# mirsadm/motioncam-decoder

Hardware: AMD Instinct MI355X
Metric: MPixels/s unpacked + achieved HBM GB/s %peak, 4K 12-bit, 1/2/4/8 GPUs (higher is better)
Workload: dtype u16; 1 GPU; 3840x2160 12-bit type-7 x 240 frames/GPU, Nat (smooth field + noise sigma 12); frames_per_gpu=240, width=3840, height=2160, bits=12, encoding=7, streams=1

## Files before the change

### motioncam_decoder_amd/csrc/mcraw_dev.h

```cpp
#pragma once
#include <hip/hip_runtime.h>
#include <stdint.h>

#include "mcraw_plan.h"

namespace mcraw {

typedef unsigned short u16x2 __attribute__((ext_vector_type(2)));

__device__ __forceinline__ uint32_t len7_of(uint32_t b)
{
    return b <= 6u ? 8u * b : (b <= 8u ? 64u : (b <= 10u ? 80u : 128u));
}

__device__ __forceinline__ uint32_t cls7_of(uint32_t b)
{
    return b <= 6u ? b : (b <= 8u ? 7u : (b <= 10u ? 8u : 9u));
}

__device__ __forceinline__ uint32_t byte_mask(uint32_t g)
{
    return __builtin_amdgcn_perm(0u, 0u, 0x0C0C0C0Cu + g);
}

// ... 110 lines not shown

__device__ __forceinline__ void post_pack12(const uint32_t p[4], uint32_t o[3])
{
    uint32_t t[4];
#pragma unroll
    for (int i = 0; i < 4; i++) {
        const uint32_t c = __builtin_bit_cast(uint32_t, __builtin_elementwise_min(__builtin_bit_cast(mcraw_u16x2, p[i]),
                                                                                  __builtin_bit_cast(mcraw_u16x2, 0x0FFF0FFFu)));
        t[i] = __builtin_amdgcn_udot2(__builtin_bit_cast(mcraw_u16x2, c), __builtin_bit_cast(mcraw_u16x2, 0x00011000u), 0u, false);
    }
    o[0] = __builtin_amdgcn_perm(t[1], t[0], 0x06000102u);
    o[1] = __builtin_amdgcn_perm(t[2], t[1], 0x05060001u);
    o[2] = __builtin_amdgcn_perm(t[3], t[2], 0x04050600u);
}

__device__ __forceinline__ void post_pack12_lean(const uint32_t p[4], uint32_t o[3])
{
    uint32_t t[4];
#pragma unroll
    for (int i = 0; i < 4; i++)
        t[i] = __builtin_amdgcn_udot2(__builtin_bit_cast(mcraw_u16x2, p[i]), __builtin_bit_cast(mcraw_u16x2, 0x00011000u), 0u, false);
    o[0] = __builtin_amdgcn_perm(t[1], t[0], 0x06000102u);
    o[1] = __builtin_amdgcn_perm(t[2], t[1], 0x05060001u);
    o[2] = __builtin_amdgcn_perm(t[3], t[2], 0x04050600u);
}

template <int B, bool CLAMP>
__device__ __forceinline__ void post_pack_be(const uint32_t p[4], uint32_t o[4])
{
    static_assert(B == 10 || B == 14, "strip rows of 10 or 14 bits per sample");
    constexpr uint32_t MAXV = (1u << B) - 1u;
    uint32_t g[4];
#pragma unroll
    for (int i = 0; i < 4; i++) {
        uint32_t c = p[i];
        if (CLAMP)
            c = __builtin_bit_cast(uint32_t, __builtin_elementwise_min(__builtin_bit_cast(mcraw_u16x2, c), __builtin_bit_cast(mcraw_u16x2, MAXV | (MAXV << 16))));
        g[i] = __builtin_amdgcn_udot2(__builtin_bit_cast(mcraw_u16x2, c), __builtin_bit_cast(mcraw_u16x2, 0x00010000u | (1u << B)), 0u, false);
    }
    uint32_t w[4];
    if (B == 10) {
        w[0] = (g[0] << 12) | (g[1] >> 8);
        w[1] = (g[1] << 24) | (g[2] << 4) | (g[3] >> 16);
        w[2] = g[3] << 16;
        w[3] = 0u;
    } else {
        w[0] = (g[0] << 4) | (g[1] >> 24);
        w[1] = (g[1] << 8) | (g[2] >> 20);
        w[2] = (g[2] << 12) | (g[3] >> 16);
        w[3] = g[3] << 16;
    }
#pragma unroll
    for (int i = 0; i < 4; i++)
        o[i] = __builtin_amdgcn_perm(w[i], w[i], 0x00010203u);
}

#define MCRAW_GLOBAL __attribute__((address_space(1)))
template <class V, class T>
__device__ __forceinline__ MCRAW_GLOBAL V *gptr(T *p)
{
    return (MCRAW_GLOBAL V *)p;
}

#ifndef MCRAW_STORE_POLICY
#define MCRAW_STORE_POLICY "sc1 nt"
#endif
typedef uint32_t mcraw_u32x4 __attribute__((ext_vector_type(4)));
typedef uint32_t mcraw_u32x3 __attribute__((ext_vector_type(3)));
#if defined(__HIP_DEVICE_COMPILE__) && !defined(__gfx950__) && !defined(__gfx942__)
#error "store_stream16/12: the `sc1 nt` mnemonics and the two wait states behind a store of more than 8 bytes are gfx940+ facts"
#endif
__device__ __forceinline__ void store_stream16(void *dst, mcraw_u32x4 v)
{
    asm volatile("global_store_dwordx4 %0, %1, off " MCRAW_STORE_POLICY "\n\ts_nop 1" ::"v"(dst), "v"(v) : "memory");
}
__device__ __forceinline__ void store_stream12(void *dst, mcraw_u32x3 v)
{
    asm volatile("global_store_dwordx3 %0, %1, off " MCRAW_STORE_POLICY "\n\ts_nop 1" ::"v"(dst), "v"(v) : "memory");
}
typedef uint32_t mcraw_u32x2 __attribute__((ext_vector_type(2)));
__device__ __forceinline__ void store_stream8(void *dst, mcraw_u32x2 v)
{
    asm volatile("global_store_dwordx2 %0, %1, off " MCRAW_STORE_POLICY ::"v"(dst), "v"(v) : "memory");
}

enum StorePath {
    SP_ALIGNED,
    SP_UNALIGNED,
    SP_CROPPED,
    SP_MERGED_FWD,
    SP_MERGED_BACK,
};
#ifndef MCRAW_STORE_PATH
#define MCRAW_STORE_PATH(form, cond)
#endif

__device__ __forceinline__ void post_store_bytes(uint8_t *dst, const uint32_t *o, uint32_t nb, uint32_t last, uint32_t maxb)
{
    for (uint32_t i = 0; i < maxb; i++)
        if (i < nb) {
            uint32_t b = (o[i >> 2] >> (8u * (i & 3u))) & 0xffu;
            if (i == nb - 1u)
                b &= last;
            gptr<uint8_t>(dst)[i] = static_cast<uint8_t>(b);
        }
}

template <bool NT, int PB>
__device__ __forceinline__ void post_store8(uint16_t *out, const Post &post, uint32_t width, uint32_t y, uint32_t x,
                                            uint32_t p[4], uint32_t n, bool quick, bool lean = false)
{
    if (!(PB != 16 && lean) && (post.mode & POST_BLACK))
        post_black(p, post, y);
    if (PB == 10 || PB == 14) {
        constexpr uint32_t B = PB == 10 ? 10u : 14u;
        uint32_t o[4];
        if (lean)
            post_pack_be<(PB == 10 ? 10 : 14), false>(p, o);
        else
            post_pack_be<(PB == 10 ? 10 : 14), true>(p, o);
        uint8_t *dst = reinterpret_cast<uint8_t *>(out) + static_cast<size_t>(y) * post_row_bytes(width, post.mode) + (x >> 3) * B;
        if (quick && n == 8u) {
            MCRAW_STORE_PATH(SP_ALIGNED, true);
            typedef uint32_t u32x2_u __attribute__((ext_vector_type(2), aligned(2)));
            typedef uint32_t u32x3_u __attribute__((ext_vector_type(3), aligned(2)));
            if (PB == 10) {
                const u32x2_u v = {o[0], o[1]};
                *gptr<u32x2_u>(dst) = v;
                *gptr<uint16_t>(dst + 8) = static_cast<uint16_t>(o[2]);
            } else {
                const u32x3_u v = {o[0], o[1], o[2]};
                *gptr<u32x3_u>(dst) = v;
                *gptr<uint16_t>(dst + 12) = static_cast<uint16_t>(o[3]);
            }
        } else {
            MCRAW_STORE_PATH(SP_UNALIGNED, n == 8u);
            MCRAW_STORE_PATH(SP_CROPPED, n != 8u);
            const uint32_t bitsn = n * B, nb = (bitsn + 7u) >> 3;
            post_store_bytes(dst, o, nb, (bitsn & 7u) ? (0xffu << (8u - (bitsn & 7u))) & 0xffu : 0xffu, 14u);
        }
        return;
    }
    if (PB == 12) {
        uint32_t o[3];
        if (lean)
            post_pack12_lean(p, o);
        else
            post_pack12(p, o);
        uint8_t *dst = reinterpret_cast<uint8_t *>(out) + static_cast<size_t>(y) * post_row_bytes(width, post.mode) + (x >> 3) * 12u;
        if (quick && n == 8u) {
            MCRAW_STORE_PATH(SP_ALIGNED, true);
            typedef uint32_t u32x3 __attribute__((ext_vector_type(3), aligned(4)));
            const u32x3 v = {o[0], o[1], o[2]};
            if (NT)
                store_stream12(dst, v);
            else
                *gptr<u32x3>(dst) = v;
        } else if (n == 8u) {
            MCRAW_STORE_PATH(SP_UNALIGNED, true);
            typedef uint32_t u32x3_u __attribute__((ext_vector_type(3), aligned(1)));
            const u32x3_u v = {o[0], o[1], o[2]};
            *gptr<u32x3_u>(dst) = v;
        } else {
            MCRAW_STORE_PATH(SP_CROPPED, true);
            const uint32_t nb = (n * 12u + 7u) >> 3;
#pragma unroll
// ... 190 lines not shown
```

### motioncam_decoder_amd/csrc/mcraw_type7.hip

```cpp
#include <algorithm>
#include <cstdlib>

#if defined(MCRAW_PATHST) || defined(MCRAW_PATHS7)
#include "mcraw_census.h"
#endif
#ifdef MCRAW_PATHST
namespace mcraw {
enum PathT {
    PT_WAVES,
    PT_INVALID,
    PT_SHORT,
    PT_TILES_SKIPPED,
    PT_SPAN_EMPTY, PT_SPAN_FULL, PT_HEAD,
    PT_WG_REMAP, PT_WG_CHUNKED,
    PT_CLS0, PT_CLS9 = PT_CLS0 + 9,
    PT_PAIR_DIFF,
    PT_WRAP_LANES,
    PT_LEAN, PT_NOTLEAN,
    PT_FAIL_BITS, PT_FAIL_REF, PT_FAIL_TOP, PT_FAIL_WRAP,
    PT_DROP_Y, PT_DROP_X,
    PT_ST_ALIGNED, PT_ST_UNALIGNED, PT_ST_CROPPED,
    PT_ST_MERGED_FWD, PT_ST_MERGED_BACK,
    PT_DECL_PARTIAL, PT_DECL_NOTIN,
    PT_N
// ... 73 lines not shown
        return u;
    }
    const uint4 row = s_tab[cidx * 8u + k];
    uint32_t lo = 0, hi = 0;
    const uint32_t tms[3] = {row.x, row.y, row.z};
#pragma unroll
    for (int t = 0; t < 3; t++) {
        const uint32_t tm = tms[t];
        if (!ALIGNED8 && t > 0 && !__any(tm != 0u))
            continue;
        const uint2 p = lds_read8<ALIGNED8>(base, blk + term_off(tm));
        const uint32_t m = term_mask(tm);
        lo |= ((p.x >> term_shr(tm)) & m) << term_shl(tm);
        hi |= ((p.y >> term_shr(tm)) & m) << term_shl(tm);
    }
    const uint32_t th = row.w;
    uint32_t lo8 = 0, hi8 = 0;
    if (ALIGNED8 || __any(th != 0u)) {
        const uint2 ph = lds_read8<ALIGNED8>(base, blk + term_off(th));
        const uint32_t mh = term_mask(th);
        lo8 = (ph.x >> term_shr(th)) & mh;
        hi8 = (ph.y >> term_shr(th)) & mh;
    }
    u.x[0] = __builtin_amdgcn_perm(lo8, lo, 0x05010400u);
    u.x[1] = __builtin_amdgcn_perm(lo8, lo, 0x07030602u);
    u.x[2] = __builtin_amdgcn_perm(hi8, hi, 0x05010400u);
    u.x[3] = __builtin_amdgcn_perm(hi8, hi, 0x07030602u);
    return u;
}

#ifndef MCRAW_SIDE_T
#define MCRAW_SIDE_T 512
#endif
#ifndef MCRAW_SIDE_LPT
#define MCRAW_SIDE_LPT 4
#endif
#ifndef MCRAW_SIDE_LCAP
#define MCRAW_SIDE_LCAP 512
#endif
#ifndef MCRAW_SPEC_WARM
#define MCRAW_SPEC_WARM 8192
#endif
constexpr uint32_t SIDE_XL = 9;
constexpr uint32_t SIDE_OUT = 0xFFu;
constexpr uint32_t SIDE_DEAD = 0xFEu;
static_assert(ITEM_SPLIT == 2, "k7_side sums the block lengths of half a record per item");

template <int PATTERN>
__device__ __forceinline__ uint32_t swz_xor(uint32_t v)
{
    return static_cast<uint32_t>(__builtin_amdgcn_ds_swizzle(static_cast<int>(v), PATTERN));
}

__device__ __forceinline__ void lds_barrier()
{
    asm volatile("s_waitcnt lgkmcnt(0)\n\ts_barrier" ::: "memory");
}

__device__ __forceinline__ uint2 side_strides(const uint4 v, uint32_t odd)
{
    const uint32_t pick = odd ? 0x07050301u : 0x06040200u;
    uint32_t st[2];
#pragma unroll
    for (int i = 0; i < 2; i++) {
        const uint32_t h4 = i ? __builtin_amdgcn_perm(v.w, v.z, pick) : __builtin_amdgcn_perm(v.y, v.x, pick);
        const uint32_t hb = (h4 >> 4) & 0x0F0F0F0Fu;
        const uint32_t sel = hb & 0x07070707u;
        const uint32_t lo = __builtin_amdgcn_perm(0x08060504u, 0x03020100u, sel);
        const uint32_t hi = __builtin_amdgcn_perm(0x10101010u, 0x100A0A08u, sel);
        const uint32_t g = (hb >> 3) & 0x01010101u;
        const uint32_t m = byte_mask(g);
        st[i] = (((hi & m) | (lo & ~m)) << 2) + 0x01010101u;
    }
    return make_uint2(st[0], st[1]);
}

#ifdef MCRAW_DIAG
#ifndef SIDE_PROF_BLOCK
#define SIDE_PROF_BLOCK 1u
#endif
__device__ unsigned long long g_side_prof[2][256];
#define SIDE_STAMP(slot)                                                                                               \
    do {                                                                                                               \
        if (blockIdx.x == SIDE_PROF_BLOCK && (tid == 0u || tid == 64u) && tl_n_ < 255u) {                              \
            const unsigned long long now_ = __builtin_amdgcn_s_memtime();                                              \
            g_side_prof[tid ? 1 : 0][++tl_n_] = (static_cast<unsigned long long>(slot) << 48) | (now_ - stamp_);       \
            g_side_prof[tid ? 1 : 0][0] = tl_n_;                                                                        \
        }                                                                                                              \
    } while (0)
#else
#define SIDE_STAMP(slot)
#endif

#ifdef MCRAW_PATHS7
enum Path7 {
    P7_STREAMS, P7_REJECTED,
    P7_RECORDS,
    P7_UNITS, P7_UNITS_FULL, P7_PIECE_STEPS, P7_UNITS_DEAD, P7_SKIPPED_UNITS,
    P7_DEAD,
    P7_RUN_PASSES, P7_RUN_PASSES64,
    P7_SEGW_SWITCH,
    P7_SEGW_PIECES, P7_SEGW_REPAIRED, P7_SEGW_ROUNDS2,
    P7_SEGW_RESUMED,
    P7_PARTS, P7_PART_EMPTY, P7_COUNTED, P7_SPEC,
    P7_HO_MUTE, P7_HO_OVER, P7_HO_PASS, P7_HO_LAST, P7_HO_HIT, P7_HO_MISS,
    P7_HO_MUTE_WORK, P7_HO_MUTE_PART1,
    P7_LASTC_REPLAYED,
    P7_REPLAY_UNITS, P7_REPLAY_PIECEFLAG,
    P7_REPLAY_TAIL,
    P7_TOLD_LATE,
    P7_ITEMS_BEHIND_PART0, P7_TRUNCATED_BY_TILES,
    P7_N
};
__device__ unsigned long long g_k7_paths[P7_N];
#define K7_PATH(slot, v) (p7_[slot] += static_cast<uint32_t>(v))
#else
#define K7_PATH(slot, v)
#endif

template <uint32_t SIDE_T, uint32_t SIDE_LPT, uint32_t SIDE_LCAP, uint32_t SPEC_WARM, bool PARTS, bool LASTC>
__global__ __launch_bounds__(SIDE_T) __attribute__((amdgpu_waves_per_eu(4, 4))) void k7_side(const Work7 W)
{
    constexpr uint32_t SIDE_PIECE = 16 * SIDE_T * SIDE_LPT;
    constexpr uint32_t SIDE_HALF = SIDE_PIECE / 2;
    constexpr uint32_t SIDE_BYTES = SIDE_PIECE + SIDE_XL * 16 + 16;
    __shared__ __attribute__((aligned(16))) uint8_t s_b[SIDE_BYTES];
    __shared__ __attribute__((aligned(16))) uint8_t s_T[SIDE_HALF + 80];
    __shared__ __attribute__((aligned(16))) uint16_t s_L[2][SIDE_LCAP];
    __shared__ __attribute__((aligned(16))) uint16_t s_len[2][2 * SIDE_LCAP];
    __shared__ uint4 s_tab[72];
    __shared__ __attribute__((aligned(16))) uint32_t s_st[2][4];
    __shared__ uint2 s_seg[64];
    __shared__ int32_t s_err;

    const uint32_t nfr = static_cast<uint32_t>(W.n7), nsb = PARTS ? W.nsplit[0] : 1u, nsr = PARTS ? W.nsplit[1] : 1u;
    const uint32_t bq = blockIdx.x / nfr, f = blockIdx.x - bq * nfr;
    const uint32_t s = bq < nsr ? 1u : 0u, part = s ? bq : bq - nsr, nsp = s ? nsr : nsb;
    const uint32_t fs = (nsb + nsr) * f + (s ? nsb : 0u) + part;
    const uint32_t tid = threadIdx.x, lane = tid & 63u;
    const uint32_t wave = __builtin_amdgcn_readfirstlane(tid >> 6);
#ifdef MCRAW_PATHS7
    uint32_t p7_[P7_N] = {};
#endif
#ifdef MCRAW_DIAG
    const unsigned long long stamp_ = __builtin_amdgcn_s_memtime();
    uint32_t tl_n_ = 0, nsteps_ = 0;
#endif
    if (tid < 72u)
        s_tab[tid] = reinterpret_cast<const uint4 *>(c_tab7)[tid];
    if (tid < 80u)
        s_T[SIDE_HALF + tid] = static_cast<uint8_t>(SIDE_OUT);
    if (tid == 0u)
        s_err = 0;

    const Plan7 PL = W.plans[f];
    const Plan7 *P = &PL;
    int32_t *status = W.status + fs;
    const uint32_t len = P->len;
    const __amdgpu_buffer_rsrc_t rs = frame_rsrc(P->in, len);
    SIDE_STAMP(10);

    const uint4 hv = ld_b128(rs, 0);
    const uint32_t encW = __builtin_amdgcn_readfirstlane(hv.x), encH = __builtin_amdgcn_readfirstlane(hv.y);
    const uint32_t bitsOff = __builtin_amdgcn_readfirstlane(hv.z), refsOff = __builtin_amdgcn_readfirstlane(hv.w);
    const uint32_t so = s ? refsOff : bitsOff;
    const uint64_t A0 = (static_cast<uint64_t>(so) + 4u) & ~15ull;
    const uint32_t odd = (so + 4u) & 1u;
    struct Lines {
        uint4 v[SIDE_LPT], x;
    };
    auto load_piece = [&](Lines &r, uint32_t piece) {
        const uint64_t base = A0 + static_cast<uint64_t>(piece) * SIDE_PIECE;
#pragma unroll
        for (uint32_t j = 0; j < SIDE_LPT; j++) {
            const uint64_t o = base + 16ull * (tid + SIDE_T * j);
            r.v[j] = o < len ? ld_b128(rs, static_cast<uint32_t>(o)) : make_uint4(0, 0, 0, 0);
        }
        r.x = make_uint4(0, 0, 0, 0);
        if (tid < SIDE_XL) {
            const uint64_t o = base + 16ull * (SIDE_T * SIDE_LPT + tid);
            r.x = o < len ? ld_b128(rs, static_cast<uint32_t>(o)) : make_uint4(0, 0, 0, 0);
        }
    };
    Lines nx, ny;
    load_piece(nx, 0u);
    int32_t err = 0;
    uint32_t tilesX = 0, nblk = 0, R = 0;
    if (len < 16u || bitsOff > len || refsOff > len || (encW & 63u) != 0u || encW < static_cast<uint32_t>(P->width) ||
        encW == 0u || encH == 0u || (encH & 3u) != 0u ||
        static_cast<uint64_t>(encW) * encH >= (1ull << 31)) {
        err = MCRAW_E_HEADER;
    } else {
        tilesX = encW >> 6;
        nblk = 4u * tilesX * (encH >> 2);
        R = (nblk + GROUP_BLOCKS - 1u) / GROUP_BLOCKS;
        if (R > P->ngroups)
            err = E_GEOMETRY;
        else if (so + 4u > len || so + 4u < so)
            err = MCRAW_E_TRUNCATED;
        else {
            const uint32_t count = ld_u8(rs, so) | (ld_u8(rs, so + 1u) << 8) | (ld_u8(rs, so + 2u) << 16) |
                                   (ld_u8(rs, so + 3u) << 24);
            if (__builtin_amdgcn_readfirstlane(count) < nblk)
                err = MCRAW_E_SIDESTREAM;
        }
    }
    SIDE_STAMP(11);
    Frame7 *const FR = W.frames + f;
    if (s == 0u && part == 0u && tid == 0u) {
        FR->in = P->in;
        FR->out = P->out;
        FR->len = len;
        FR->width = P->width;
        FR->rows = min(static_cast<uint32_t>(P->height), encH);
        FR->tilesX = tilesX;
        FR->nblk = err ? 0u : nblk;
        FR->fast_store = P->fast_store;
        FR->encH = encH;
        FR->pstride = P->pstride;
        for (uint32_t q = err ? 0u : nsb - 1u; q < 3u; q++) {
            FR->part_item[q] = 0xFFFFFFFFu;
            FR->part_len[q] = 0u;
        }
        W.status[W.nstatus + f] = static_cast<int32_t>(encH);
    }
    if (err) {
        if (tid == 0u)
            *status = err;
// ... 166 lines not shown
            bool go;
            do {
                const uint32_t u = pu + lane * SU;
                const uint32_t code = s_T[min(u, SIDE_HALF)];
                const unsigned long long m = __ballot(code != SU);
                nb = m == 0ull ? 64u : static_cast<uint32_t>(__builtin_ctzll(m));
                take = min(nb, room - cnt);
                if (lane < take)
                    L[cnt + lane] = static_cast<uint16_t>(u);
                nxt = static_cast<uint32_t>(__builtin_amdgcn_readlane(static_cast<int>(code), static_cast<int>(nb & 63u)));
                cnt += take;
                pu += take * SU;
                go = take == nb && cnt < room && (nb == 64u || nxt < SIDE_DEAD);
                SU = (go && nb != 64u) ? nxt : SU;
                passes++;
                K7_PATH(P7_RUN_PASSES, 1u);
                K7_PATH(P7_RUN_PASSES64, nb == 64u);
                segw = go && passes >= 8u && passes * MCRAW_SEGW_RATIO > cnt;
#ifdef MCRAW_DIAG
                nsteps_++;
#endif
            } while (go && !segw);
            if (segw) {
            } else if (take < nb) {
                why = 1u;
            } else if (cnt >= room) {
                why = 1u;
                SU = (nb != 64u && nxt < SIDE_DEAD) ? nxt : 0u;
            } else {
                why = nxt == SIDE_OUT ? 2u : 3u;
                SU = 0u;
            }
            if (segw)
                seg_valid = false;
            K7_PATH(P7_SEGW_SWITCH, segw);
        } else if (!segw) {
            SU = 0u;
        }
        if (segw && pu < SIDE_HALF) {
            K7_PATH(P7_SEGW_RESUMED, !fresh && seg_valid);
            if (fresh || !seg_valid)
                seg_walk(pu);
            const uint32_t take = min(room - cnt, seg_total - seg_done);
            if (take)
                seg_list(L + cnt, take);
            seg_done += take;
            cnt += take;
            SU = 0u;
            if (seg_done == seg_total) {
                why = seg_exit == SEG_DEADX ? 3u : 2u;
                pu = seg_exit == SEG_DEADX ? 0u : seg_exit;
                seg_valid = false;
            } else {
                why = 1u;
                pu = 0u;
            }
        } else if (segw) {
            SU = 0u;
        }
        if (lane == 0u)
            *reinterpret_cast<uint4 *>(s_st[lst]) = make_uint4(pu, cnt, why, SU);
    };

    const uint32_t k = lane & 7u, sub = lane >> 3;
    const uint32_t first_cand = static_cast<uint32_t>((so + 4u) & 15u) >> 1;
    static_assert((2u * SIDE_LCAP) % 512u == 0u, "whole passes of 512 items");
    auto scan_unit = [&](uint32_t par, uint32_t n0, uint32_t cnt) {
        const uint32_t nitems = 2u * cnt;
        for (uint32_t base = 0; base < nitems; base += 512u) {
            const uint32_t i0 = base + 8u * lane;
            uint4 lv = make_uint4(0u, 0u, 0u, 0u);
            if (i0 < nitems)
                lv = *reinterpret_cast<const uint4 *>(&s_len[par][i0]);
            uint32_t a[8] = {lv.x & 0xffffu, lv.x >> 16, lv.y & 0xffffu, lv.y >> 16,
                             lv.z & 0xffffu, lv.z >> 16, lv.w & 0xffffu, lv.w >> 16};
            uint32_t mine = 0;
#pragma unroll
            for (uint32_t i = 0; i < 8u; i++) {
                a[i] = i0 + i < nitems ? a[i] : 0u;
                mine += a[i];
            }
            uint32_t utot;
            const uint32_t ex = wave_excl_scan(mine, lane, &utot);
            uint32_t o = static_cast<uint32_t>(carry) + ex;
#pragma unroll
            for (uint32_t i = 0; i < 8u; i++) {
                if (i0 + i < nitems)
                    goff[2u * n0 + i0 + i] = o;
                o += a[i];
            }
            carry += utot;
        }
    };

#ifdef MCRAW_INJECT_MUTE7
    constexpr uint32_t SPIN7 = 1u << 6;
#else
    constexpr uint32_t SPIN7 = 1u << 19;
#endif
    __shared__ uint32_t s_ask[4];
    bool told = part + 1u >= nsp;
    auto tell = [&](uint32_t count, uint32_t where) {
        if (!told && tid == 0u) {
#ifdef MCRAW_INJECT_MUTE7
            if (part != 0u)
#endif
            {
                look_put(sync, W.epoch, count);
                look_put(sync + 1, W.epoch, where);
            }
        }
        told = true;
    };
    auto ask = [&](uint32_t &count, uint32_t &where) {
        lds_barrier();
        if (tid == 0u) {
            uint32_t c = 0u, w = first_cand, ok = 1u;
            if (part) {
                ok = 0u;
                for (uint32_t spin = 0; spin < SPIN7; spin++) {
                    if (look_get(sync - 2, W.epoch, &c) && look_get(sync - 1, W.epoch, &w)) {
                        ok = 1u;
                        break;
                    }
                    __builtin_amdgcn_s_sleep(8);
                }
            }
            s_ask[0] = c;
            s_ask[1] = w;
            s_ask[2] = ok;
        }
        lds_barrier();
        count = s_ask[0];
        where = s_ask[1];
        return s_ask[2] != 0u;
    };
    auto nothing_to_decode = [&]() {
        if (tid == 0u && s == 0u && nsp > 1u) {
            if (part + 1u < nsp)
                FR->part_len[part] = 0u;
            if (part)
                FR->part_item[part - 1u] = 0xFFFFFFFFu;
        }
    };

    uint32_t run_piece = 0u, run_cand = first_cand, run_n = 0u;
    uint32_t nx_piece = 0u;
    uint32_t exitc = ENDX;
    bool go = true;
    if (nsp > 1u) {
        const bool empty = m_lo >= m_hi, lastp = part + 1u >= nsp;
        const bool owns0 = !empty && m_lo == 0u;
        const uint32_t m_chi = lastp ? np_guess : m_hi;
        const bool lastc = LASTC && lastp && !owns0 && rp_base != nullptr && m_chi > m_lo && m_chi != 0xFFFFFFFFu;
        const bool spec = !empty && !owns0 && (!lastp || lastc);
        K7_PATH(P7_PARTS, 1u);
        K7_PATH(P7_PART_EMPTY, empty);
        K7_PATH(P7_COUNTED, !empty && (!lastp || lastc));
        K7_PATH(P7_SPEC, spec);
        uint32_t entry = NOENTRY, cnt1 = 0u, exit1 = ENDX;
        bool dead1 = false;
        bool counted = false;
        if (!empty && (!lastp || lastc)) {
            counted = true;
            uint32_t spiece = 0xFFFFFFFFu;
            uint32_t cpiece = spec ? m_lo - 1u : 0u, lst = 0u;
            if (spec)
                load_piece(nx, cpiece);
            build_strides(nx, cpiece);
            load_piece(nx, cpiece + 1u);
            nx_piece = cpiece + 1u;
            lds_barrier();
// ... 81 lines not shown
            K7_PATH(P7_HO_LAST, 1u);
            K7_PATH(P7_LASTC_REPLAYED, lastc && pw == entry);
            run_piece = m_lo, run_cand = owns0 ? first_cand : pw, run_n = pn;
            if (lastc && pw == entry)
                replay_from_count();
        } else if (owns0 || pw == entry) {
            K7_PATH(P7_HO_HIT, 1u);
            const uint32_t upto = pn + cnt1;
            tell(min(upto, R), upto >= R || dead1 || exit1 == ENDX ? ENDX : exit1);
            run_piece = m_lo, run_cand = owns0 ? first_cand : entry, run_n = pn;
            replay_from_count();
        } else {
            K7_PATH(P7_HO_MISS, 1u);
            run_piece = m_lo, run_cand = pw, run_n = pn;
        }
        if (go && run_n >= R) {
            tell(run_n, ENDX);
            nothing_to_decode();
            go = false;
        }
    }

    uint32_t cur = 0;
    uint32_t prev_n = 0, prev_total = 0;
    if (go) {
    lds_barrier();
    upc = bb = tb = run_piece;
    n = run_n;
#ifdef MCRAW_FORCE_SEGW
    segw = true;
#else
    segw = false;
#endif
    seg_valid = false;
    carry = run_piece == 0u && decode_from == 0u ? 16u : 0u;
    if (nx_piece != run_piece)
        load_piece(nx, run_piece);
    store_bytes(nx);
    SIDE_STAMP(12);
    if (!rleft)
        build_strides(nx, run_piece);
    load_piece(nx, run_piece + 1u);
    load_piece(ny, run_piece + 2u);
    uint4 rq = make_uint4(0u, 0u, 0u, 0u);
    auto rfetch = [&](uint32_t at) { rq = ld_b128_nt(rsp, 2u * (at + 8u * lane)); };
    auto replay = [&](uint32_t lst, uint32_t room) {
#ifdef MCRAW_POISON_STRIDES7
        for (uint32_t i = lane; i < SIDE_HALF / 16u; i += 64u)
            reinterpret_cast<uint4 *>(s_T)[i] = make_uint4(0x01010101u * SIDE_DEAD, 0x01010101u * SIDE_DEAD, 0x01010101u * SIDE_DEAD, 0x01010101u * SIDE_DEAD);
#endif
        K7_PATH(P7_REPLAY_UNITS, 1u);
        const uint32_t n = min(room, rleft);
        const uint32_t w4[4] = {rq.x, rq.y, rq.z, rq.w};
        uint32_t mine = 8u, ment = 0u;
#pragma unroll
        for (int i = 7; i >= 0; i--) {
            const uint32_t idx = 8u * lane + static_cast<uint32_t>(i), e = (w4[i >> 1] >> (16 * (i & 1))) & 0xffffu;
            const bool hit = idx >= 1u && idx < n && (e & 0x8000u) != 0u;
            mine = hit ? static_cast<uint32_t>(i) : mine;
            ment = hit ? e : ment;
        }
        const unsigned long long m = __ballot(mine != 8u);
        uint32_t take = n, pu = 0u, why = 1u;
        if (m) {
            K7_PATH(P7_REPLAY_PIECEFLAG, 1u);
            const uint32_t fl = static_cast<uint32_t>(__builtin_ctzll(m));
            take = 8u * fl + wave_lane(mine, fl);
            pu = SIDE_HALF + (wave_lane(ment, fl) & 0x7fffu);
            why = 2u;
        } else if (n == rleft) {
            if (rdead)
                why = 3u;
            else if (rexit != ENDX)
                why = 2u, pu = SIDE_HALF + rexit;
        }
        if (8u * lane < take)
            *reinterpret_cast<uint4 *>(&s_L[lst][8u * lane]) = make_uint4(rq.x & 0x7fff7fffu, rq.y & 0x7fff7fffu, rq.z & 0x7fff7fffu, rq.w & 0x7fff7fffu);
        if (lane == 0u)
            *reinterpret_cast<uint4 *>(s_st[lst]) = make_uint4(pu, take, why, 0u);
        rfetch(rnext + take);
    };
    lds_barrier();
    SIDE_STAMP(13);
    if (wave == 0u) {
        if (rleft) {
            rfetch(0u);
            replay(0u, min(R - run_n, SIDE_LCAP / 4u));
        } else
            walk(0u, run_cand, 0u, min(R - run_n, SIDE_LCAP / 4u), true);
    }
    SIDE_STAMP(14);
    while (true) {
        lds_barrier();
        SIDE_STAMP(0);
        const uint4 st4 = *reinterpret_cast<const uint4 *>(s_st[cur]);
        const uint32_t pu = __builtin_amdgcn_readfirstlane(st4.x);
        const uint32_t total = __builtin_amdgcn_readfirstlane(st4.y);
        const uint32_t why = __builtin_amdgcn_readfirstlane(st4.z);
        const uint32_t SU = __builtin_amdgcn_readfirstlane(st4.w);
        const uint32_t npc = why == 2u ? upc + 1u : upc;
        const bool last = n + total >= R || why == 3u || npc >= m_hi;
        const bool skip = upc < decode_from;
        if (!skip && n_first == 0xFFFFFFFFu)
            n_first = n;
        K7_PATH(P7_UNITS, 1u);
        K7_PATH(P7_UNITS_FULL, why == 1u);
        K7_PATH(P7_PIECE_STEPS, why == 2u);
        K7_PATH(P7_UNITS_DEAD, why == 3u);
        K7_PATH(P7_SKIPPED_UNITS, skip);
        K7_PATH(P7_RECORDS, skip ? 0u : total);
        if (npc > upc && npc == m_hi)
            exitc = pu - SIDE_HALF;
        if (rleft) {
            rleft -= min(total, rleft);
            rnext += total;
        }
        const bool moved = upc > bb, build = !last && npc > tb && rleft == 0u;
        if (moved) {
            store_bytes(nx);
            bb = upc;
            nx = ny;
            load_piece(ny, bb + 2u);
        }
        if (build) {
            build_strides(nx, npc);
            tb = npc;
        }
        if (moved || build)
            lds_barrier();
        SIDE_STAMP(1);
        if (wave == 0u) {
            if (!last) {
                K7_PATH(P7_REPLAY_TAIL, rleft == 0u && rnext != 0u);
                if (rleft)
                    replay(cur ^ 1u, min(R - (n + total), SIDE_LCAP));
                else
                    walk(cur ^ 1u, npc > upc ? pu - SIDE_HALF : pu, SU, min(R - (n + total), SIDE_LCAP), npc > upc);
            }
            SIDE_STAMP(2);
            if (s == 0u && prev_total)
                scan_unit(cur ^ 1u, prev_n, prev_total);
            SIDE_STAMP(5);
        } else if (!skip) {
            const uint8_t *B = s_b;
            const uint16_t *L = s_L[cur];
            constexpr uint32_t STEP = (SIDE_T / 64u - 1u) * 8u;
            uint32_t q = (wave - 1u) * 8u + sub;
            uint32_t ro_n = q < total ? 2u * L[q] + odd : 0u;
            uint32_t hd_n = *reinterpret_cast<const uint16_t *>(B + (ro_n & ~1u)) | (static_cast<uint32_t>(B[(ro_n & ~1u) + 2u]) << 16);
            for (uint32_t qb = (wave - 1u) * 8u; qb < total; qb += STEP, q += STEP) {
                const bool live = q < total;
                const uint32_t ro = ro_n;
                const uint32_t hd = hd_n >> (8u * (ro & 1u));
                ro_n = q + STEP < total ? 2u * L[q + STEP] + odd : 0u;
                hd_n = *reinterpret_cast<const uint16_t *>(B + (ro_n & ~1u)) | (static_cast<uint32_t>(B[(ro_n & ~1u) + 2u]) << 16);
                const uint32_t b0 = live ? hd & 0xffu : 0u, b1 = (hd >> 8) & 0xffu;
                const uint32_t hb = b0 >> 4, ref = ((b0 & 15u) << 8) | b1;
                Unpacked U = unpack8<false>(B, ro + 2u, cls7_of(hb), k, s_tab);
                const u16x2 rr = __builtin_bit_cast(u16x2, ref | (ref << 16));
#pragma unroll
                for (int i = 0; i < 4; i++)
                    U.x[i] = __builtin_bit_cast(uint32_t, __builtin_bit_cast(u16x2, U.x[i]) + rr);
                const uint32_t r = n + q;
                const uint32_t idx = r * 64u + 8u * k;
                if (s == 1u) {
                    if (live)
                        *reinterpret_cast<uint4 *>(refs + idx) = make_uint4(U.x[0], U.x[1], U.x[2], U.x[3]);
                    continue;
                }
                const uint32_t nvalid = live ? min(8u, nblk - min(nblk, idx)) : 0u;
                if (nvalid < 8u) {
#pragma unroll
                    for (uint32_t i = 0; i < 4u; i++)
                        U.x[i] &= nvalid >= 2u * i + 2u ? 0xffffffffu : nvalid == 2u * i + 1u ? 0xffffu : 0u;
                }
                uint32_t c[4], over = 0;
#pragma unroll
                for (uint32_t i = 0; i < 4u; i++) {
                    c[i] = __builtin_bit_cast(uint32_t, __builtin_elementwise_min(__builtin_bit_cast(u16x2, U.x[i]),
                                                                                  __builtin_bit_cast(u16x2, 0x00100010u)));
                    over |= c[i] ^ U.x[i];
                }
                if (over)
                    lane_err |= MCRAW_E_SIDESTREAM;
                const uint32_t bytes_lo = __builtin_amdgcn_perm(c[1], c[0], 0x06040200u);
                const uint32_t bytes_hi = __builtin_amdgcn_perm(c[3], c[2], 0x06040200u);
                if (live)
                    *reinterpret_cast<uint2 *>(bits + idx) = make_uint2(bytes_lo, bytes_hi);
                uint32_t l8 = 0;
#pragma unroll
                for (uint32_t i = 0; i < 2u; i++) {
                    const uint32_t v4 = i ? bytes_hi : bytes_lo;
                    const uint32_t sel = v4 & 0x07070707u;
                    const uint32_t lo = __builtin_amdgcn_perm(0x08060504u, 0x03020100u, sel);
                    const uint32_t hi = __builtin_amdgcn_perm(0x10101010u, 0x100A0A08u, sel);
                    const uint32_t g = (v4 >> 3) & 0x01010101u;
                    const uint32_t m = byte_mask(g);
                    const uint32_t l4 = ((hi & m) | (lo & ~m)) | (v4 & 0x10101010u);
                    l8 = __builtin_amdgcn_sad_u8(l4, 0u, l8);
                }
                l8 += swz_xor<0x041F>(l8);
                l8 += swz_xor<0x081F>(l8);
                if (live && (k & 3u) == 0u)
                    s_len[cur][2u * q + (k >> 2)] = static_cast<uint16_t>(l8 << 3);
            }
            SIDE_STAMP(3);
        }
        prev_n = n;
        prev_total = skip ? 0u : total;
        n += total;
        if (last) {
            dead = why == 3u && n < R && !skip;
            break;
        }
        upc = npc;
        cur ^= 1u;
    }
    K7_PATH(P7_TOLD_LATE, !told);
    K7_PATH(P7_DEAD, dead);
    tell(min(n, R), n >= R || dead || exitc == ENDX ? ENDX : exitc);
    if (s == 0u && prev_total) {
        lds_barrier();
        if (wave == 0u)
            scan_unit(cur, prev_n, prev_total);
    }
    if (tid == 0u) {
        if (dead)
            lane_err |= MCRAW_E_TRUNCATED;
        if (s == 0u) {
            const uint32_t c32 = static_cast<uint32_t>(min(carry, static_cast<uint64_t>(0xffffffffu)));
            if (n >= R && !dead && n_first != 0xFFFFFFFFu) {
                goff[ITEM_SPLIT * R] = c32;
                if (nsp == 1u && carry > len)
                    lane_err |= MCRAW_E_TRUNCATED;
            }
            if (nsp > 1u) {
                if (part + 1u < nsp)
                    FR->part_len[part] = n_first != 0xFFFFFFFFu ? c32 : 0u;
                if (part)
                    FR->part_item[part - 1u] = n_first != 0xFFFFFFFFu ? ITEM_SPLIT * n_first : 0xFFFFFFFFu;
            }
        }
    }
    }
#ifdef MCRAW_PATHS7
    if (tid == 0u)
        for (uint32_t i = 0; i < P7_N; i++)
            if (p7_[i])
                atomicAdd(&g_k7_paths[i], static_cast<unsigned long long>(p7_[i]));
#endif
    if (lane_err)
        atomicOr(&s_err, lane_err);
    lds_barrier();
    if (tid == 0u)
        *status = s_err;
    SIDE_STAMP(15);
#ifdef MCRAW_DIAG
    if (blockIdx.x == SIDE_PROF_BLOCK && tid == 0u)
        g_side_prof[0][255] = nsteps_;
#endif
}

constexpr int PAY_LDS = ITEM_SPAN + 16 + 32;
constexpr uint32_t PAY_CHUNKS = ITEM_SPAN / 16 + 1;

struct ItemS {
    uint32_t valid;
    uint32_t g, nblk, tilesX;
    uint32_t base16, n16, head;
    int32_t width, rows;
    uint32_t fast;
    const uint8_t *in;
    uint32_t len;
    uint16_t *out;
    size_t meta;
    uint32_t lean;
    uint32_t pstride;
};

__device__ __forceinline__ ItemS item_scalars(const Work7 &W, uint32_t item, uint32_t first_frame, uint32_t class_groups)
{
    ItemS I;
    const uint32_t per = W.Rmax * ITEM_SPLIT;
    const uint32_t cper = class_groups * ITEM_SPLIT;
    const uint32_t fc = item / cper;
    const uint32_t f = first_frame + fc;
    const uint32_t g = item - fc * cper;
    const Frame7 *F = W.frames + f;
    const uint32_t nblk = F->nblk;
    const uint32_t *grp = W.grp_off + static_cast<size_t>(f) * (per + 1u) + g;
    I.valid = g * ITEM_BLOCKS < nblk ? 1u : 0u;
    uint32_t start = 0, end = 0;
    if (I.valid) {
        start = grp[0];
        end = grp[1];
        if (W.nsplit[0] > 1u) {
            uint32_t ps = 0u, pe = 0u, sum_s = 0u;
            uint64_t e64 = end;
#pragma unroll
            for (uint32_t q = 0; q < 3u; q++) {
                const uint32_t pi = F->part_item[q];
                ps = g >= pi ? q + 1u : ps;
                pe = g + 1u >= pi && pi != 0xFFFFFFFFu ? q + 1u : pe;
            }
#pragma unroll
            for (uint32_t q = 0; q < 3u; q++) {
                const uint32_t pl = F->part_len[q];
                sum_s += q < ps ? pl : 0u;
                e64 += q < pe ? pl : 0u;
            }
            start += sum_s;
            end = static_cast<uint32_t>(e64);
#ifdef MCRAW_PATHS7
            if ((threadIdx.x & 63u) == 0u) {
                if (ps > 0u)
                    atomicAdd(&g_k7_paths[P7_ITEMS_BEHIND_PART0], 1ull);
                if ((g + 1u) * ITEM_BLOCKS >= nblk && e64 > F->len)
                    atomicAdd(&g_k7_paths[P7_TRUNCATED_BY_TILES], 1ull);
            }
#endif
            if ((g + 1u) * ITEM_BLOCKS >= nblk && e64 > F->len)
                atomicOr(W.status + (W.nsplit[0] + W.nsplit[1]) * f, MCRAW_E_TRUNCATED);
        }
    }
    I.g = g;
    I.nblk = nblk;
    I.tilesX = F->tilesX;
    I.base16 = start & ~15u;
    I.head = start - I.base16;
    I.n16 = I.valid ? min((end - min(end, I.base16) + 15u) >> 4, PAY_CHUNKS) : 0u;
    I.width = F->width;
    I.rows = static_cast<int32_t>(F->rows);
    I.fast = F->fast_store;
    I.in = F->in;
    I.len = F->len;
    I.out = F->out;
    I.meta = static_cast<size_t>(f) * W.Rmax * 64u + static_cast<size_t>(g) * ITEM_BLOCKS;
    I.lean = 0u;
    I.pstride = F->pstride;
#ifdef MCRAW_FORCE_SLOWSTORET
    I.fast = 0u;
#endif
// ... 322 lines not shown
```

Baseline: 1.946 million MPixels/s.

## Use sc1 cache-policy stores for side-stream outputs and set wave priorities

```diff
diff --git a/motioncam_decoder_amd/csrc/mcraw_dev.h b/motioncam_decoder_amd/csrc/mcraw_dev.h
--- a/motioncam_decoder_amd/csrc/mcraw_dev.h
+++ b/motioncam_decoder_amd/csrc/mcraw_dev.h
@@ -216,6 +216,22 @@
 __device__ __forceinline__ void store_stream8(void *dst, mcraw_u32x2 v)
 {
     asm volatile("global_store_dwordx2 %0, %1, off " MCRAW_STORE_POLICY ::"v"(dst), "v"(v) : "memory");
+}
+
+#ifndef MCRAW_WT_POLICY
+#define MCRAW_WT_POLICY "sc1"
+#endif
+__device__ __forceinline__ void store_wt16(void *dst, mcraw_u32x4 v)
+{
+    asm volatile("global_store_dwordx4 %0, %1, off " MCRAW_WT_POLICY "\n\ts_nop 1" ::"v"(dst), "v"(v) : "memory");
+}
+__device__ __forceinline__ void store_wt8(void *dst, mcraw_u32x2 v)
+{
+    asm volatile("global_store_dwordx2 %0, %1, off " MCRAW_WT_POLICY ::"v"(dst), "v"(v) : "memory");
+}
+__device__ __forceinline__ void store_wt4(void *dst, uint32_t v)
+{
+    asm volatile("global_store_dword %0, %1, off " MCRAW_WT_POLICY ::"v"(dst), "v"(v) : "memory");
 }
 
 enum StorePath {
diff --git a/motioncam_decoder_amd/csrc/mcraw_type7.hip b/motioncam_decoder_amd/csrc/mcraw_type7.hip
--- a/motioncam_decoder_amd/csrc/mcraw_type7.hip
+++ b/motioncam_decoder_amd/csrc/mcraw_type7.hip
@@ -179,7 +179,7 @@
 __device__ unsigned long long g_side_prof[2][256];
 #define SIDE_STAMP(slot)                                                                                               \
     do {                                                                                                               \
-        if (blockIdx.x == SIDE_PROF_BLOCK && (tid == 0u || tid == 64u) && tl_n_ < 255u) {                              \
+        if (blockIdx.x == SIDE_PROF_BLOCK && (tid == 0u || tid == 64u) && tl_n_ < 253u) {                              \
             const unsigned long long now_ = __builtin_amdgcn_s_memtime();                                              \
             g_side_prof[tid ? 1 : 0][++tl_n_] = (static_cast<unsigned long long>(slot) << 48) | (now_ - stamp_);       \
             g_side_prof[tid ? 1 : 0][0] = tl_n_;                                                                        \
@@ -240,7 +240,7 @@
     uint32_t p7_[P7_N] = {};
 #endif
 #ifdef MCRAW_DIAG
-    const unsigned long long stamp_ = __builtin_amdgcn_s_memtime();
+    const unsigned long long stamp_ = __builtin_amdgcn_s_memtime(), rstamp_ = __builtin_amdgcn_s_memrealtime();
     uint32_t tl_n_ = 0, nsteps_ = 0;
 #endif
     if (tid < 72u)
@@ -573,12 +573,21 @@
             }
             uint32_t utot;
             const uint32_t ex = wave_excl_scan(mine, lane, &utot);
-            uint32_t o = static_cast<uint32_t>(carry) + ex;
+            uint32_t o = static_cast<uint32_t>(carry) + ex, ov[8];
 #pragma unroll
             for (uint32_t i = 0; i < 8u; i++) {
-                if (i0 + i < nitems)
-                    goff[2u * n0 + i0 + i] = o;
+                ov[i] = o;
                 o += a[i];
+            }
+            uint32_t *const gp = goff + 2u * n0 + i0;
+            if (i0 + 8u <= nitems) {
+                store_wt16(gp, mcraw_u32x4{ov[0], ov[1], ov[2], ov[3]});
+                store_wt16(gp + 4, mcraw_u32x4{ov[4], ov[5], ov[6], ov[7]});
+            } else {
+#pragma unroll
+                for (uint32_t i = 0; i < 8u; i++)
+                    if (i0 + i < nitems)
+                        store_wt4(gp + i, ov[i]);
             }
             carry += utot;
         }
@@ -826,6 +835,15 @@
     };
     lds_barrier();
     SIDE_STAMP(13);
+    if constexpr (!PARTS) {
+        if (s == 0u) {
+            if (wave == 0u)
+                __builtin_amdgcn_s_setprio(3);
+            else
+                __builtin_amdgcn_s_setprio(2);
+        } else if (wave == 0u)
+            __builtin_amdgcn_s_setprio(1);
+    }
     if (wave == 0u) {
         if (rleft) {
             rfetch(0u);
@@ -909,7 +927,7 @@
                 const uint32_t idx = r * 64u + 8u * k;
                 if (s == 1u) {
                     if (live)
-                        *reinterpret_cast<uint4 *>(refs + idx) = make_uint4(U.x[0], U.x[1], U.x[2], U.x[3]);
+                        store_wt16(refs + idx, mcraw_u32x4{U.x[0], U.x[1], U.x[2], U.x[3]});
                     continue;
                 }
                 const uint32_t nvalid = live ? min(8u, nblk - min(nblk, idx)) : 0u;
@@ -930,7 +948,7 @@
                 const uint32_t bytes_lo = __builtin_amdgcn_perm(c[1], c[0], 0x06040200u);
                 const uint32_t bytes_hi = __builtin_amdgcn_perm(c[3], c[2], 0x06040200u);
                 if (live)
-                    *reinterpret_cast<uint2 *>(bits + idx) = make_uint2(bytes_lo, bytes_hi);
+                    store_wt8(bits + idx, mcraw_u32x2{bytes_lo, bytes_hi});
                 uint32_t l8 = 0;
 #pragma unroll
                 for (uint32_t i = 0; i < 2u; i++) {
@@ -974,7 +992,7 @@
         if (s == 0u) {
             const uint32_t c32 = static_cast<uint32_t>(min(carry, static_cast<uint64_t>(0xffffffffu)));
             if (n >= R && !dead && n_first != 0xFFFFFFFFu) {
-                goff[ITEM_SPLIT * R] = c32;
+                store_wt4(goff + ITEM_SPLIT * R, c32);
                 if (nsp == 1u && carry > len)
                     lane_err |= MCRAW_E_TRUNCATED;
             }
@@ -1000,8 +1018,11 @@
         *status = s_err;
     SIDE_STAMP(15);
 #ifdef MCRAW_DIAG
-    if (blockIdx.x == SIDE_PROF_BLOCK && tid == 0u)
+    if (blockIdx.x == SIDE_PROF_BLOCK && tid == 0u) {
         g_side_prof[0][255] = nsteps_;
+        g_side_prof[1][254] = __builtin_amdgcn_s_memtime() - stamp_;
+        g_side_prof[1][255] = __builtin_amdgcn_s_memrealtime() - rstamp_;
+    }
 #endif
 }
 
```

Result: no change. 1.968 million MPixels/s, median of 6 (+1.2%).
